# domanovi/FEC_Erasure_Code_Unit_Test_Relay

Hardware: AMD Instinct MI355X
Metric: GiB/s device-resident erasure encode+decode, 300B pkts, T=10; %HBM roofline (higher is better)
Workload: dtype u8; 1 GPU; encode 1000010 + decode 1000000 x 300B packets per GPU, one stream per GPU, (T,B,N)=(10,3,3); T=10, B=3, N=3, packets_per_gpu=1000000

## Files before the change

fec_erasure_code_unit_test_relay_amd/_lib.py:

```python
from __future__ import annotations

import ctypes
import os

_HERE = os.path.dirname(os.path.abspath(__file__))
LIB_PATH = os.environ.get("FEC_AMD_LIB") or os.path.join(_HERE, "libfec_amd.so")
HEADER_PATHS = [os.path.join(_HERE, "..", "include", "fec_amd.h")]

FEC_OK = 0
FEC_ERR_ARG = -1
FEC_ERR_HIP = -2
FEC_ERR_NOMEM = -3
FEC_ERR_WORKSPACE = -4
FEC_ERR_SEQUENCE = -5
FEC_ERR_HISTORY = -6

KERNEL_NAMES = ["fec_encode_kernel", "fec_scan_kernel", "fec_plan_kernel", "fec_copy_kernel",
                "fec_recover_kernel"]


class FecError(RuntimeError):
    def __init__(self, status: int, what: str = ""):
        msg = lib().fec_strerror(status).decode() if _lib is not None else str(status)
        if status == FEC_ERR_HIP and _lib is not None:
# ... 6 lines not shown

_lib = None


def lib() -> ctypes.CDLL:
    global _lib
    if _lib is not None:
        return _lib
    if not os.path.exists(LIB_PATH):
        raise RuntimeError(
            f"{LIB_PATH} is missing: the HIP extension must be built first "
            "(make -C fec_erasure_code_unit_test_relay_amd/csrc); there is no fallback")
    try:
        import torch
    except ImportError:
        pass
    L = ctypes.CDLL(LIB_PATH)
    vp, i32, i64 = ctypes.c_void_p, ctypes.c_int, ctypes.c_int64
    ip = ctypes.POINTER(ctypes.c_int)
    i64p = ctypes.POINTER(ctypes.c_int64)
    L.fec_strerror.restype = ctypes.c_char_p
    L.fec_strerror.argtypes = [i32]
    L.fec_last_error.restype = i32
    L.fec_last_error.argtypes = [ctypes.c_char_p, ctypes.c_size_t]
    L.fec_version.restype = i32
    L.fec_codec_create.argtypes = [i32, i32, i32, i32, ctypes.POINTER(vp)]
    L.fec_codec_destroy.argtypes = [vp]
    L.fec_codec_geometry.argtypes = [vp, ip, ip, ip, ip]
    L.fec_codec_generator.argtypes = [vp, vp]
    L.fec_codec_set_encode_path.argtypes = [vp, i32]
    L.fec_encode_tile_fetch.argtypes = [i32, i32, i32, i32, i32, ip, ip, ip, ip]
    L.fec_codec_set_copy_path.argtypes = [vp, i32]
    L.fec_codec_set_plan_path.argtypes = [vp, i32]
    L.fec_codec_info.argtypes = [vp, ctypes.c_char_p, ctypes.c_size_t]
    L.fec_codec_set_episode_dedup.argtypes = [vp, i32]
    L.fec_debug_stamps.argtypes = [vp, i32, vp]
    L.fec_encode_batch.argtypes = [vp, vp, vp, i64, i64, vp, vp, vp]
    L.fec_decode_workspace_bytes.restype = ctypes.c_size_t
    L.fec_decode_workspace_bytes.argtypes = [vp, i64]
    L.fec_decode_batch.argtypes = [vp, vp, vp, i64, vp, vp, vp, ctypes.c_size_t, vp]
    L.fec_decode_counters.argtypes = [vp, i64p, i64p, i64p]
    L.fec_streams_create.argtypes = [i32, i32, i32, i32, i32, ctypes.POINTER(vp)]
    L.fec_streams_destroy.argtypes = [vp]
    L.fec_streams_encode.argtypes = [vp, vp, i32, vp, vp, vp, vp, vp]
    L.fec_streams_decode.argtypes = [vp, vp, i32, vp, vp, vp, vp, vp]
    L.fec_streams_state.argtypes = [vp, i32, i64p, i64p]
    L.fec_streams_encode_burst.argtypes = [vp, vp, vp, i32, vp, vp, vp, vp, vp]
    L.fec_streams_decode_burst.argtypes = [vp, vp, vp, i32, vp, vp, vp, vp, vp]
    L.fec_streams_plan_burst_host.argtypes = [i32, i32, i32, i32, vp, vp, i32, vp]
    L.fec_streams_create_mixed.argtypes = [i32, vp, i32, vp, i32, ctypes.POINTER(vp)]
    L.fec_streams_codes.argtypes = [vp, ip, ip]
    L.fec_streams_stream_geometry.argtypes = [vp, i32, ip, ip, ip, ip, ip, ip]
    L.fec_streams_set_code.argtypes = [vp, i32, i32]
    L.fec_streams_mixed_fit.argtypes = [i32, vp, i32, vp, vp, vp, vp]
    L.fec_decode_stream_create.argtypes = [ctypes.POINTER(vp)]
    L.fec_decode_stream_destroy.argtypes = [vp]
    L.fec_decode_stream_state.argtypes = [vp, i64p, i64p]
    L.fec_decode_stream_push.argtypes = [vp, vp, vp, vp, vp, i64, i64, vp, vp, i64p, vp, ctypes.c_size_t, vp]
    L.fec_decode_plan_stats.argtypes = [vp, i64p, i64p]
    L.fec_decode_plan.argtypes = [vp, vp, i64, vp, ctypes.c_size_t, vp]
    L.fec_decode_apply.argtypes = [vp, vp, vp, i64, vp, vp, vp, ctypes.c_size_t, vp]
    L.fec_decode_copy.argtypes = [vp, vp, vp, i64, vp, vp, vp]
    L.fec_decode_recover.argtypes = [vp, vp, i64, vp, vp, vp, ctypes.c_size_t, vp]
    L.fec_timing_enable.argtypes = [vp, i32]
    L.fec_timing_collect.argtypes = [vp, ctypes.POINTER(ctypes.c_double), i64p]
    L.fec_encoder_create.argtypes = [i32, i32, i32, i32, ctypes.POINTER(vp)]
# ... 119 lines not shown
```

fec_erasure_code_unit_test_relay_amd/codec.py:

```python
from __future__ import annotations

import ctypes

import numpy as np

from ._lib import KERNEL_NAMES, check, lib


def _stream_handle(torch):
    return ctypes.c_void_p(torch.cuda.current_stream().cuda_stream)


def _ptr(t):
    return ctypes.c_void_p(t.data_ptr()) if t is not None else None


def _check_out(torch, out, out_len, rows: int, width: int, device):
    if out is None:
        out = torch.empty((rows, width), dtype=torch.uint8, device=device)
    else:
        assert out.dtype == torch.uint8 and out.is_cuda and out.is_contiguous(), "out: contiguous uint8 GPU tensor"
        assert out.dim() == 2 and out.shape[1] == width and out.shape[0] >= rows, \
            f"out must be at least [{rows}, {width}], got {tuple(out.shape)}"
    if out_len is None:
# ... 14 lines not shown
class Codec:

    def __init__(self, max_payload: int, T: int, B: int, N: int):
        h = ctypes.c_void_p()
        check(lib().fec_codec_create(max_payload, T, B, N, ctypes.byref(h)), "fec_codec_create")
        self._h = h
        v = [ctypes.c_int() for _ in range(4)]
        check(lib().fec_codec_geometry(h, *[ctypes.byref(x) for x in v]), "fec_codec_geometry")
        self.k, self.n, self.S, self.CW = (x.value for x in v)
        self.L, self.T, self.B, self.N = max_payload, T, B, N
        self._ws = None

    def __del__(self):
        if getattr(self, "_h", None) and lib is not None:
            try:
                lib().fec_codec_destroy(self._h)
            except Exception:
                pass
            self._h = None

    def generator(self) -> np.ndarray:
        G = np.zeros(self.k * self.n, dtype=np.uint8)
        check(lib().fec_codec_generator(self._h, G.ctypes.data_as(ctypes.c_void_p)), "generator")
        return G.reshape(self.k, self.n)

    def set_encode_path(self, path: str) -> None:
        code = {"auto": 0, "generic": 1, "tile": 5}[path]
        check(lib().fec_codec_set_encode_path(self._h, code), "fec_codec_set_encode_path")

    def set_copy_path(self, path: str) -> None:
        code = {"auto": 0, "generic": 1, "fast": 2}[path]
        check(lib().fec_codec_set_copy_path(self._h, code), "fec_codec_set_copy_path")

    def info(self) -> dict:
        import json
        buf = ctypes.create_string_buffer(512)
        check(lib().fec_codec_info(self._h, buf, 512), "fec_codec_info")
        return json.loads(buf.value.decode())

    def set_plan_path(self, path: str) -> None:
        code = {"auto": 0, "generic": 1, "fast": 2}[path]
        check(lib().fec_codec_set_plan_path(self._h, code), "fec_codec_set_plan_path")

    def set_episode_dedup(self, on: bool) -> None:
        check(lib().fec_codec_set_episode_dedup(self._h, int(bool(on))), "fec_codec_set_episode_dedup")

    def encode_blocks(self, data, out=None):
        import torch
        assert data.dtype == torch.uint8 and data.is_cuda and data.dim() == 2 and data.shape[1] == self.k
        data = data.contiguous()
        if out is None:
            out = torch.empty((data.shape[0], self.n), dtype=torch.uint8, device=data.device)
        check(lib().fec_block_encode_batch(self._h, _ptr(data), data.shape[0], _ptr(out), _stream_handle(torch)),
              "fec_block_encode_batch")
        return out

    def decode_blocks(self, cw, erasure):
        import torch
        assert cw.dtype == torch.uint8 and cw.is_cuda and cw.dim() == 2 and cw.shape[1] == self.n
        assert erasure.dtype == torch.uint8 and erasure.shape == cw.shape
        cw, erasure = cw.contiguous(), erasure.contiguous()
        out = torch.empty_like(cw)
        er_out = torch.empty_like(erasure)
        check(lib().fec_block_decode_batch(self._h, _ptr(cw), _ptr(erasure), cw.shape[0], _ptr(out), _ptr(er_out),
                                           _stream_handle(torch)), "fec_block_decode_batch")
        return out, er_out

    def encode(self, payload, lengths=None, history: int = 0, out=None, out_len=None):
        import torch
        assert payload.dtype == torch.uint8 and payload.is_cuda and payload.dim() == 2
# ... 353 lines not shown
```

fec_erasure_code_unit_test_relay_amd/csrc/fec_codec.hip:

```cpp
#include <hip/hip_runtime.h>
#include <hip/hip_ext.h>

#include <algorithm>
#include <atomic>
#include <chrono>
#include <functional>
#include <cstdio>
#include <cstdlib>
#include <cstring>
#include <memory>
#include <mutex>
#include <new>
#include <vector>

#include "fec_amd.h"
#include "fec_host.h"
#include "fec_kernels.h"
#include "fec_status.h"

using fec::Geometry;

namespace {

constexpr int kLdsBudget = 64 * 1024;
constexpr int kCopyLdsBudget = 32 * 1024;
constexpr int kMaxPayload = 1500;

inline int round16(int v) { return (v + 15) & ~15; }

#define HIP_TRY(expr)                                  \
    do {                                               \
        if ((expr) != hipSuccess) return FEC_ERR_HIP;  \
    } while (0)

struct EventPair {
    int kernel;
    hipEvent_t a, b;
};

}

struct fec_decode_stream {
    int64_t consumed = 0;
    int64_t last_cut = 0;
};

struct fec_codec {
    Geometry g;
    bool compact_fresh = false;
    std::vector<uint8_t> G;
    std::shared_ptr<const fec::DecodeRules> rules;
    uint32_t* d_ptab = nullptr;
    uint8_t* d_rules = nullptr;
    int64_t* d_wbase = nullptr;
    uint8_t* d_rules_log = nullptr;
    const void* plan_fast = nullptr;
    uint8_t* d_gf = nullptr;
    uint8_t* d_G = nullptr;
    uint8_t* d_rstate = nullptr;
    int enc_tp = 0;
    int encode_path = 0;
    int cus = 0;
    const void* tile_kernel = nullptr;
    fec::TileGeom tile{};
    int tile_per_cu = 0;
    const void* copy_fast = nullptr;
    int copyf_tp = 0;
    int copy_path = 0;
    int plan_path = 0;
    int dedup = 1;
    uint64_t* d_stamps = nullptr;
    int stamp_kernel = -1;
    int copy_tp = 0;
    bool timing = false;
    std::vector<EventPair> events;
    hipStream_t side = nullptr;
    hipEvent_t ev_fork = nullptr, ev_join = nullptr;

    ~fec_codec() {
        if (ev_fork) (void)hipEventDestroy(ev_fork);
        if (ev_join) (void)hipEventDestroy(ev_join);
        if (side) (void)hipStreamDestroy(side);
        for (auto& e : events) {
            (void)hipEventDestroy(e.a);
            (void)hipEventDestroy(e.b);
        }
        if (d_ptab) (void)hipFree(d_ptab);
        if (d_rules) (void)hipFree(d_rules);
        if (d_wbase) (void)hipFree(d_wbase);
        if (d_rules_log) (void)hipFree(d_rules_log);
        if (d_gf) (void)hipFree(d_gf);
        if (d_G) (void)hipFree(d_G);
        if (d_rstate) (void)hipFree(d_rstate);
    }

    int enc_lds(int tp) const {
        const int SP = (g.S + 3) & ~3;
        const int rows = tp + g.n - 1;
        const int Sk = g.S * g.k;
        return round16(g.k * rows * SP) + round16(tp * g.CW) + 2 * ((Sk + 7) & ~7) + 4 * rows;
    }
    int copy_lds(int tp) const { return round16(tp * g.CW) + 2 * ((g.L + 2 + 7) & ~7) + 4 * tp; }
// ... 383 lines not shown
    ca.CW = g.CW;
    ca.T = g.T;
    ca.TP = c->copy_tp;
    ca.cwt_bytes = round16(ca.TP * g.CW);
    const int64_t cblocks = (Pout + ca.TP - 1) / ca.TP;
    hipEvent_t stop;
    if (int st = c->begin(FEC_KERNEL_DEC_COPY, s, &stop)) return st;
    hipLaunchKernelGGL(fec::fec_copy_kernel, dim3(static_cast<unsigned>(cblocks)), dim3(256),
                       c->copy_lds(ca.TP), s, ca);
    HIP_TRY(hipGetLastError());
    return c->end(stop, s);
}

int launch_compact(fec_codec* c, int64_t P, void* d_ws, size_t ws_bytes, hipStream_t s) {
    const Geometry& g = c->g;
    if (P - g.T <= 0) return FEC_OK;
    if (int st = check_ws(c, P, d_ws, ws_bytes)) return st;
    const Ws w = ws_carve(g, P, d_ws);
    fec::CompactArgs ca;
    ca.counters = w.counters;
    ca.erased = w.erased;
    ca.src_d = w.src_d;
    ca.sym_ok = w.sym_ok;
    ca.k = g.k;
    ca.rec_list = w.rec_list;
    if (!c->compact_fresh)
        HIP_TRY(hipMemsetAsync(w.counters + 2, 0, 4, s));
    c->compact_fresh = false;
    hipLaunchKernelGGL(fec::fec_compact_kernel, dim3(256), dim3(256), 0, s, ca);
    HIP_TRY(hipGetLastError());
    return FEC_OK;
}

int launch_recover(fec_codec* c, const uint8_t* d_cw, int64_t P, uint8_t* d_out, int32_t* d_outlen,
                   void* d_ws, size_t ws_bytes, hipStream_t s, int64_t row_off = 0, bool compacted = false) {
    const Geometry& g = c->g;
    const int64_t Pout = P - g.T;
    if (Pout <= 0) return FEC_OK;
    if (int st = check_ws(c, P, d_ws, ws_bytes)) return st;
    if (!compacted)
        if (int st = launch_compact(c, P, d_ws, ws_bytes, s)) return st;
    const Ws w = ws_carve(g, P, d_ws);
    fec::RecArgs ra;
    ra.cw = d_cw;
    ra.P = P;
    ra.Pout = Pout;
    ra.counters = w.counters;
    ra.rec_list = w.rec_list;
    ra.coef = w.coef;
    ra.gf = c->d_gf;
    ra.out = d_out;
    ra.out_len = d_outlen;
    ra.L = g.L;
    ra.k = g.k;
    ra.n = g.n;
    ra.S = g.S;
    ra.CW = g.CW;
    hipEvent_t stop;
    if (int st = c->begin(FEC_KERNEL_DEC_RECOVER, s, &stop)) return st;
    ra.row_off = row_off;
    ra.stamps = (c->stamp_kernel == FEC_KERNEL_DEC_RECOVER) ? c->d_stamps : nullptr;
    const int span = (g.k + g.n - 1) * g.CW + 32;
    ra.stage_bytes = (span <= 12 * 1024 && g.n <= 17) ? ((span + 15) & ~15) : 0;
    const unsigned rgrid = static_cast<unsigned>(std::min<int64_t>((Pout + 3) / 4, 1024));
    const int maxn = g.n <= 17 ? 17 : 32;
    const int lds = fec::recover_lds_bytes(maxn, ra.stage_bytes);
    if (g.n > 17)
        hipLaunchKernelGGL((fec::fec_recover_kernel_t<32, false>), dim3(rgrid), dim3(256), lds, s, ra);
    else if (ra.stage_bytes)
        hipLaunchKernelGGL((fec::fec_recover_kernel_t<17, true>), dim3(rgrid), dim3(256), lds, s, ra);
    else
        hipLaunchKernelGGL((fec::fec_recover_kernel_t<17, false>), dim3(rgrid), dim3(256), lds, s, ra);
    HIP_TRY(hipGetLastError());
    return c->end(stop, s);
}

int launch_decode(fec_codec* c, const uint8_t* d_cw, const uint8_t* d_er, int64_t P, uint8_t* d_out,
                  int32_t* d_outlen, void* d_ws, size_t ws_bytes, hipStream_t s) {
    if (P - c->g.T <= 0) return FEC_OK;
    if (int st = check_ws(c, P, d_ws, ws_bytes)) return st;
    HIP_TRY(hipEventRecord(c->ev_fork, s));
    HIP_TRY(hipStreamWaitEvent(c->side, c->ev_fork, 0));
    if (int st = launch_plan(c, d_er, P, d_ws, ws_bytes, c->side)) return st;
    if (int st = launch_compact(c, P, d_ws, ws_bytes, c->side)) return st;
    HIP_TRY(hipEventRecord(c->ev_join, c->side));
    if (int st = launch_copy(c, d_cw, d_er, P, d_out, d_outlen, s)) return st;
    HIP_TRY(hipStreamWaitEvent(s, c->ev_join, 0));
    return launch_recover(c, d_cw, P, d_out, d_outlen, d_ws, ws_bytes, s, 0, true);
}

int launch_decode_stream(fec_codec* c, fec_decode_stream* st, const uint8_t* d_cw, const uint8_t* d_er,
                         const uint8_t* h_er, int64_t P, int64_t history, uint8_t* d_out, int32_t* d_outlen,
                         int64_t* n_out, void* d_ws, size_t ws_bytes, hipStream_t s) {
    const int T = c->g.T;
// ... 300 lines not shown
    if (!c || P < 0) return FEC_ERR_ARG;
    if (P > c->g.T && (!d_cw || !d_out || !d_outlen)) return FEC_ERR_ARG;
    return launch_recover(c, d_cw, P, d_out, d_outlen, d_ws, ws_bytes,
                          static_cast<hipStream_t>(stream));
}

int fec_decode_counters(const void* d_ws, int64_t* episodes, int64_t* recovered, int64_t* lost) {
    if (!d_ws) return FEC_ERR_ARG;
    int32_t h[8];
    HIP_TRY(hipDeviceSynchronize());
    HIP_TRY(hipMemcpy(h, d_ws, sizeof(h), hipMemcpyDeviceToHost));
    if (episodes) *episodes = h[6] + h[7];
    if (recovered) *recovered = h[2];
    if (lost) *lost = h[1] - h[2];
    return FEC_OK;
}

int fec_codec_info(const fec_codec* c, char* buf, size_t size) {
    if (!c || !buf || size == 0) return FEC_ERR_ARG;
    char enc[64];
    const int np = c->g.n - c->g.k;
    if (c->tile_kernel && (c->encode_path == 0 || c->encode_path == 5))
        std::snprintf(enc, sizeof(enc), "fec_encode_tile_kernel<%d, %d, %d, false>", c->g.k, np,
                      c->tile_kernel == fec::fec_encode_tile_kernel_for(c->g.k, np, 0) ? 0 : c->g.L);
    else
        std::snprintf(enc, sizeof(enc), "fec_encode_kernel");
    char cpy[64];
    if (c->copy_path != 1 && copy_pair_kernel(c))
        std::snprintf(cpy, sizeof(cpy), "fec_copy_pair_kernel<%d, %d>", c->g.k, np);
    else if (c->copy_fast && c->copy_path != 1)
        std::snprintf(cpy, sizeof(cpy), "fec_copy_fast_kernel<%d, %d>", c->g.k, np);
    else
        std::snprintf(cpy, sizeof(cpy), "fec_copy_kernel");
    std::snprintf(buf, size,
                  "{\"k\": %d, \"n\": %d, \"S\": %d, \"CW\": %d, \"encode_kernel\": \"%s\", "
                  "\"copy_kernel\": \"%s\", \"encode_tile_packets\": %d, \"encode_tile_workgroups_per_cu\": %d, "
                  "\"copy_tile\": %d, \"plan_specialised\": %d}",
                  c->g.k, c->g.n, c->g.S, c->g.CW, enc, cpy, c->tile.R, c->tile_per_cu, c->copyf_tp,
                  c->plan_fast ? 1 : 0);
    return FEC_OK;
}

int fec_decode_plan_stats(const void* d_ws, int64_t* replayed, int64_t* filled) {
    if (!d_ws) return FEC_ERR_ARG;
    int32_t h[8];
    HIP_TRY(hipDeviceSynchronize());
    HIP_TRY(hipMemcpy(h, d_ws, sizeof(h), hipMemcpyDeviceToHost));
    if (replayed) *replayed = h[6];
    if (filled) *filled = h[7];
    return FEC_OK;
}

int fec_debug_stamps(fec_codec* c, int kernel, void* d_stamps) {
    if (!c) return FEC_ERR_ARG;
    c->stamp_kernel = d_stamps ? kernel : -1;
    c->d_stamps = static_cast<uint64_t*>(d_stamps);
    return FEC_OK;
}

int fec_codec_set_episode_dedup(fec_codec* c, int on) {
    if (!c) return FEC_ERR_ARG;
    c->dedup = on ? 1 : 0;
    return FEC_OK;
}

int fec_codec_set_plan_path(fec_codec* c, int path) {
    if (!c || path < 0 || path > 2) return FEC_ERR_ARG;
    if (path == 2 && !c->plan_fast) return FEC_ERR_ARG;
    c->plan_path = path;
    return FEC_OK;
}

int fec_codec_set_copy_path(fec_codec* c, int path) {
    if (!c || path < 0 || path > 2) return FEC_ERR_ARG;
    if (path == 2 && !c->copy_fast) return FEC_ERR_ARG;
    c->copy_path = path;
    return FEC_OK;
}

int fec_codec_set_encode_path(fec_codec* c, int path) {
    if (!c || !(path == 0 || path == 1 || path == 5)) return FEC_ERR_ARG;
    if (path == 5 && !c->tile_kernel) return FEC_ERR_ARG;
    c->encode_path = path;
    return FEC_OK;
}

int fec_encode_tile_fetch(int max_payload, int T, int B, int N, int seg, int* R, int* issued, int* live_body,
                          int* live_front) {
    if (max_payload < 0 || T < 0 || B < 0 || N < 0 || N > T) return FEC_ERR_ARG;
    const int L = max_payload, k = T - N + 1, np = B, n = k + np;
    const fec::TileGeom tg = fec::tile_geometry(k, np, L, seg != 0);
    const bool have = (L & 3) == 0 && tg.ok &&
                      (seg ? fec::fec_encode_tile_seg_kernel_for(k, np, L) : fec::fec_encode_tile_kernel_for(k, np, L));
    int body = 0, front = 0;
    if (have) {
        const int CPR = (L + 15) >> 4;
        for (int c = 0; c < tg.ngl * 256; ++c) {
            body += fec::tile_piece_live(tg.R, CPR, n, c, false);
            front += np > 0 && fec::tile_piece_live(tg.R, CPR, n, c, true);
        }
    }
    if (R) *R = have ? tg.R : 0;
    if (issued) *issued = have ? tg.ngl * 256 : 0;
    if (live_body) *live_body = body;
    if (live_front) *live_front = front;
    return have ? 1 : 0;
}

int fec_timing_enable(fec_codec* c, int enable) {
    if (!c) return FEC_ERR_ARG;
// ... 615 lines not shown
```

fec_erasure_code_unit_test_relay_amd/csrc/fec_copy_fast.hip:

```cpp
#include "fec_device.h"
#include "fec_kernels.h"

namespace fec {

template <int K, int NP>
__device__ __forceinline__ void copy_tile_convert(const CopyFastArgs& a, int64_t x0, int ntile, int delta,
                                                  const uint8_t* raw, uint8_t* xo, int32_t* clen, const uint8_t* erw) {
    constexpr int n = K + NP;
    const int tid = threadIdx.x, NT = blockDim.x;
    const int L = a.L, CW = a.CW, NS4 = a.NS4, T = a.T;
    for (int t = tid; t < ntile; t += NT) {
        int ln = 0, copy = 0;
        if (!erw[t]) {
            const uint8_t* row = raw + delta + t * CW;
            const int hdr = row[0] * 256 + row[(1 / K) * n + 1 % K];
            bool slow = false;
            for (int d = 0; d <= T; ++d) slow = slow || erw[t + d];
            ln = slow ? min(hdr, L) : hdr;
            copy = min(ln, L);
        }
        clen[t] = copy;
        a.out_len[x0 + t] = ln;
    }
    __syncthreads();
// ... 99 lines not shown
            if (lo >= delta && lo + 16 <= total) *reinterpret_cast<uint4*>(raw + lo) = v[q];
        }
        if (tid == 0) {
            for (int b = delta; b < total && (b & 3); ++b) raw[b] = gA[b];
            for (int b = total & ~3; b < total && b >= ((delta + 3) & ~3); ++b) raw[b] = gA[b];
        }
        for (int o = tid * 4; o < 32; o += 256 * 4) {
            const int lo16 = delta & ~15, hi16 = total & ~15;
            const int oa = lo16 + o, ob = hi16 + (o - 16);
            if (o < 16 && oa >= delta && oa + 4 <= total && !(lo16 >= delta && lo16 + 16 <= total))
                *reinterpret_cast<uint32_t*>(raw + oa) = *reinterpret_cast<const uint32_t*>(gA + oa);
            if (o >= 16 && ob >= delta && ob + 4 <= total && hi16 != lo16)
                *reinterpret_cast<uint32_t*>(raw + ob) = *reinterpret_cast<const uint32_t*>(gA + ob);
        }
        for (int i = tid; i < ntile + T; i += 256) erw[i] = a.er[x0 + i];
    };
    const int64_t xa = static_cast<int64_t>(blockIdx.x) * 2 * a.TP, xb = xa + a.TP;
    const int na = static_cast<int>(min<int64_t>(a.TP, a.Pout - xa));
    const int nb = static_cast<int>(max<int64_t>(0, min<int64_t>(a.TP, a.Pout - xb)));
    const int da = static_cast<int>(reinterpret_cast<uintptr_t>(a.cw + xa * CW) & 15);
    const int db = static_cast<int>(reinterpret_cast<uintptr_t>(a.cw + xb * CW) & 15);
    load(xa, na, da);
    land(xa, na, da);
    __syncthreads();
    if (nb > 0) load(xb, nb, db);
    copy_tile_convert<K, NP>(a, xa, na, da, raw, xo, clen, erw);
    if (nb <= 0) return;
    __syncthreads();
    land(xb, nb, db);
    __syncthreads();
    copy_tile_convert<K, NP>(a, xb, nb, db, raw, xo, clen, erw);
}

#define FEC_COPY_FAST_LIST(X) \
    X(8, 3) X(9, 5) X(11, 0) X(10, 1) X(9, 2) X(7, 4) X(6, 5) X(5, 6) X(4, 7) X(3, 8) X(2, 9)  \
    X(1, 10) X(10, 3) X(9, 3) X(10, 4) X(8, 4) X(10, 5) X(7, 5) X(3, 9)

#define FEC_COPY_FAST_INST(K, NP) \
    template __global__ void fec_copy_fast_kernel<K, NP>(CopyFastArgs); \
    template __global__ void fec_copy_pair_kernel<K, NP>(CopyFastArgs);
FEC_COPY_FAST_LIST(FEC_COPY_FAST_INST)

const void* fec_copy_pair_kernel_for(int k, int np) {
#define FEC_COPY_PAIR_CASE(K, NP) \
    if (k == K && np == NP) return reinterpret_cast<const void*>(&fec_copy_pair_kernel<K, NP>);
    FEC_COPY_FAST_LIST(FEC_COPY_PAIR_CASE)
#undef FEC_COPY_PAIR_CASE
    return nullptr;
}

const void* fec_copy_fast_kernel_for(int k, int np) {
#define FEC_COPY_FAST_CASE(K, NP) \
    if (k == K && np == NP) return reinterpret_cast<const void*>(&fec_copy_fast_kernel<K, NP>);
    FEC_COPY_FAST_LIST(FEC_COPY_FAST_CASE)
#undef FEC_COPY_FAST_CASE
    return nullptr;
}

}
```

fec_erasure_code_unit_test_relay_amd/csrc/fec_kernels.h:

```cpp
#pragma once

#include <hip/hip_runtime.h>
#include <cstddef>
#include <stdint.h>

namespace fec {

struct EncArgs {
    const uint8_t* payload;
    const int32_t* len;
    int64_t history;
    int64_t P;
    uint8_t* cw;
    int32_t* cw_len;
    const uint32_t* ptab;
    int L, k, n, S, CW;
    int SP;
    int TP;
    int ROWS;
    int plane;
    int xin_bytes, xout_bytes;
};

struct TileGeom {
// ... 80 lines not shown
struct EncMultiArgs {
    const uint8_t* payload;
    const int32_t* len;
    const uint32_t* gtab;
    const int64_t* seg;
    uint8_t* cur_rows;
    uint8_t* old_rows;
    int32_t* cur_len;
    int32_t* old_len;
    int L;
    int ntuple;
    int tkey[kEncMultiMax];
    int tfirst[kEncMultiMax + 1];
    int toff[kEncMultiMax];
    int nt;
    int ncf;
    int cf_first;
};
bool fec_encode_tile_multi_supports(int k, int np, int L);
const void* fec_encode_tile_multi_kernel_ptr();

struct CopyFastArgs {
    const uint8_t* cw;
    const uint8_t* er;
    int64_t P, Pout;
    uint8_t* out;
    int32_t* out_len;
    int L, CW, NS4, T, TP;
    int raw_bytes;
    int out_bytes;
    uint64_t* stamps;
};

const void* fec_copy_fast_kernel_for(int k, int np);
constexpr int kPairQ = 6;
const void* fec_copy_pair_kernel_for(int k, int np);
const void* fec_plan_fast_kernel_for(int k, int np);

struct CopyArgs {
    const uint8_t* cw;
    const uint8_t* er;
    int64_t P, Pout;
    uint8_t* out;
    int32_t* out_len;
    int L, k, n, S, CW, T, TP;
    int cwt_bytes;
};

constexpr int kPlanMaxN = 31;

struct PlanArgs {
    const uint8_t* er;
    int64_t P, Pout;
    const uint8_t* rules;
    const uint8_t* G;
    int64_t wbase[kPlanMaxN + 1];
    const uint8_t* gf;
    int ES;
    int k, n, T;
    const int32_t* counters;
    const int32_t* work;
    const int32_t* dups;
    const uint64_t* keys;
    const int32_t* reps_tr;
    int32_t* src_d;
    const uint8_t* rstate;
// ... 26 lines not shown
    uint64_t* stamps;
};
__global__ void fec_episode_kernel(EpisodeArgs a);

struct CompactArgs {
    int32_t* counters;
    const int32_t* erased;
    const int32_t* src_d;
    const uint8_t* sym_ok;
    int k;
    int32_t* rec_list;
};
__global__ void fec_compact_kernel(CompactArgs a);

struct RecArgs {
    const uint8_t* cw;
    int64_t P, Pout;
    const int32_t* counters;
    const int32_t* rec_list;
    const uint8_t* coef;
    const uint8_t* gf;
    uint8_t* out;
    int32_t* out_len;
    int L, k, n, S, CW;
    int64_t row_off;
    int stage_bytes;
    uint64_t* stamps;
};
inline int recover_lds_bytes(int maxn, int stage_bytes) {
    return 1552 + 4 * (((2 * 16 * maxn + 15) & ~15) + stage_bytes);
}
template <int MAXN, bool STAGED>
__global__ void fec_recover_kernel_t(RecArgs a);


struct BlockArgs {
    const uint8_t* in;
    const uint8_t* er;
    uint8_t* out;
    uint8_t* er_out;
    int64_t nblk;
    int k, n;
    const uint8_t* G;
    const uint8_t* gf;
    const uint8_t* rules;
    int64_t wbase_n;
    int ES;
};
__global__ void fec_block_encode_kernel(BlockArgs a);

struct CodecView {
    int L, T, B, N, k, n, S, CW;
    const uint8_t* G;
    const uint8_t* gf;
    const uint8_t* rules;
    int64_t wbase_n;
    int ES;
    const uint32_t* ptab;
};
__global__ void fec_block_decode_kernel(BlockArgs a);

__global__ void fec_encode_kernel(EncArgs a);
__global__ void fec_plan_kernel(PlanArgs a);
__global__ void fec_copy_kernel(CopyArgs a);

__global__ void fec_fill_kernel(uint8_t* out, int64_t t0, int64_t count, int L, uint64_t seed);
// ... 54 lines not shown
```

include/fec_amd.h:

```cpp
#ifndef FEC_AMD_H
#define FEC_AMD_H

#include <stddef.h>
#include <stdint.h>

#ifdef __cplusplus
extern "C" {
#endif

#define FEC_OK 0
#define FEC_ERR_ARG (-1)
#define FEC_ERR_HIP (-2)
#define FEC_ERR_NOMEM (-3)
#define FEC_ERR_WORKSPACE (-4)
#define FEC_ERR_SEQUENCE (-5)
#define FEC_ERR_HISTORY (-6)

typedef struct fec_codec fec_codec;
typedef struct fec_encoder fec_encoder;
typedef struct fec_decoder fec_decoder;

#define FEC_AMD_ABI_VERSION 2

const char *fec_strerror(int status);
int fec_last_error(char *buf, size_t size);
int fec_version(void);

int fec_codec_create(int max_payload, int T, int B, int N, fec_codec **out);
int fec_codec_destroy(fec_codec *codec);
int fec_codec_geometry(const fec_codec *codec, int *k, int *n, int *S, int *CW);
int fec_codec_info(const fec_codec *codec, char *buf, size_t size);
int fec_codec_set_encode_path(fec_codec *codec, int path);
int fec_encode_tile_fetch(int max_payload, int T, int B, int N, int seg, int *R, int *issued, int *live_body,
                          int *live_front);
int fec_codec_set_copy_path(fec_codec *codec, int path);
int fec_codec_set_plan_path(fec_codec *codec, int path);
int fec_codec_set_episode_dedup(fec_codec *codec, int on);
int fec_codec_generator(const fec_codec *codec, uint8_t *G);

int fec_encode_batch(fec_codec *codec, const uint8_t *d_payload, const int32_t *d_payload_len,
                     int64_t history, int64_t P, uint8_t *d_codeword, int32_t *d_codeword_len,
                     void *hip_stream);

size_t fec_decode_workspace_bytes(const fec_codec *codec, int64_t P);
int fec_decode_batch(fec_codec *codec, const uint8_t *d_codeword, const uint8_t *d_erasure,
                     int64_t P, uint8_t *d_payload_out, int32_t *d_payload_len, void *d_workspace,
                     size_t workspace_bytes, void *hip_stream);
typedef struct fec_decode_stream fec_decode_stream;
int fec_decode_stream_create(fec_decode_stream **out);
int fec_decode_stream_destroy(fec_decode_stream *st);
int fec_decode_stream_push(fec_codec *codec, fec_decode_stream *st, const uint8_t *d_codeword,
                           const uint8_t *d_erasure, const uint8_t *h_erasure, int64_t P, int64_t history,
                           uint8_t *d_payload_out, int32_t *d_payload_len, int64_t *n_out,
                           void *d_workspace, size_t workspace_bytes, void *hip_stream);
int fec_decode_stream_state(const fec_decode_stream *st, int64_t *consumed, int64_t *last_cut);
int fec_decode_plan(fec_codec *codec, const uint8_t *d_erasure, int64_t P, void *d_workspace,
                    size_t workspace_bytes, void *hip_stream);
int fec_decode_apply(fec_codec *codec, const uint8_t *d_codeword, const uint8_t *d_erasure,
                     int64_t P, uint8_t *d_payload_out, int32_t *d_payload_len, void *d_workspace,
                     size_t workspace_bytes, void *hip_stream);
int fec_decode_copy(fec_codec *codec, const uint8_t *d_codeword, const uint8_t *d_erasure,
                    int64_t P, uint8_t *d_payload_out, int32_t *d_payload_len, void *hip_stream);
int fec_decode_recover(fec_codec *codec, const uint8_t *d_codeword, int64_t P,
                       uint8_t *d_payload_out, int32_t *d_payload_len, void *d_workspace,
                       size_t workspace_bytes, void *hip_stream);
int fec_decode_counters(const void *d_workspace, int64_t *episodes, int64_t *recovered,
                        int64_t *lost);
int fec_decode_plan_stats(const void *d_ws, int64_t *replayed, int64_t *filled);
// ... 204 lines not shown
```

Baseline: 979.7 GiB/s.

## Add specialised one-wave-per-row erasure recover kernel with LDS staging and GF tables

Adds a templated fast recover kernel, specialised per (k, n-k). Each 64-lane wave stages one recovered row's codeword span into LDS with 16-byte vector loads, prefetches the next row's indices, and builds per-coefficient nibble multiply tables in LDS. It then computes four output bytes per lane with packed GF(256) table multiplies and writes the output with aligned 32-bit stores. The aim is to cut the per-byte gather and GF multiply cost of the generic recover kernel. In exchange it adds template instantiations and only applies when the span fits the staging buffer. The generic path stays selectable.

```diff
diff --git a/fec_erasure_code_unit_test_relay_amd/_lib.py b/fec_erasure_code_unit_test_relay_amd/_lib.py
--- a/fec_erasure_code_unit_test_relay_amd/_lib.py
+++ b/fec_erasure_code_unit_test_relay_amd/_lib.py
@@ -62,6 +62,12 @@
     L.fec_encode_tile_fetch.argtypes = [i32, i32, i32, i32, i32, ip, ip, ip, ip]
     L.fec_codec_set_copy_path.argtypes = [vp, i32]
     L.fec_codec_set_plan_path.argtypes = [vp, i32]
+    L.fec_codec_set_recover_path.argtypes = [vp, i32]
+    L.fec_codec_set_recover_path.restype = i32
+    L.fec_recover_fast_items.argtypes = [i32, i32, i32, i32, i64, i64, vp, vp, vp]
+    L.fec_recover_fast_items.restype = i32
+    L.fec_recover_fast_mul.argtypes = [ctypes.c_uint32, ctypes.c_uint32]
+    L.fec_recover_fast_mul.restype = ctypes.c_uint32
     L.fec_codec_info.argtypes = [vp, ctypes.c_char_p, ctypes.c_size_t]
     L.fec_codec_set_episode_dedup.argtypes = [vp, i32]
     L.fec_debug_stamps.argtypes = [vp, i32, vp]
diff --git a/fec_erasure_code_unit_test_relay_amd/codec.py b/fec_erasure_code_unit_test_relay_amd/codec.py
--- a/fec_erasure_code_unit_test_relay_amd/codec.py
+++ b/fec_erasure_code_unit_test_relay_amd/codec.py
@@ -70,10 +70,14 @@
         code = {"auto": 0, "generic": 1, "fast": 2}[path]
         check(lib().fec_codec_set_copy_path(self._h, code), "fec_codec_set_copy_path")
 
+    def set_recover_path(self, path: str) -> None:
+        code = {"auto": 0, "generic": 1, "fast": 2}[path]
+        check(lib().fec_codec_set_recover_path(self._h, code), "fec_codec_set_recover_path")
+
     def info(self) -> dict:
         import json
-        buf = ctypes.create_string_buffer(512)
-        check(lib().fec_codec_info(self._h, buf, 512), "fec_codec_info")
+        buf = ctypes.create_string_buffer(1024)
+        check(lib().fec_codec_info(self._h, buf, 1024), "fec_codec_info")
         return json.loads(buf.value.decode())
 
     def set_plan_path(self, path: str) -> None:
diff --git a/fec_erasure_code_unit_test_relay_amd/csrc/fec_codec.hip b/fec_erasure_code_unit_test_relay_amd/csrc/fec_codec.hip
--- a/fec_erasure_code_unit_test_relay_amd/csrc/fec_codec.hip
+++ b/fec_erasure_code_unit_test_relay_amd/csrc/fec_codec.hip
@@ -16,6 +16,7 @@
 #include "fec_amd.h"
 #include "fec_host.h"
 #include "fec_kernels.h"
+#include "fec_recover_fast.h"
 #include "fec_status.h"
 
 using fec::Geometry;
@@ -68,6 +69,7 @@
     int copyf_tp = 0;
     int copy_path = 0;
     int plan_path = 0;
+    int recover_path = 0;
     int dedup = 1;
     uint64_t* d_stamps = nullptr;
     int stamp_kernel = -1;
@@ -517,6 +519,11 @@
     return FEC_OK;
 }
 
+const void* recover_fast_kernel(const Geometry& g) {
+    if (fec::rec_fast_span_max(g.k, g.n, g.CW) > fec::kRecFastStageMax) return nullptr;
+    return fec::fec_recover_fast_kernel_for(g.k, g.n - g.k);
+}
+
 int launch_recover(fec_codec* c, const uint8_t* d_cw, int64_t P, uint8_t* d_out, int32_t* d_outlen,
                    void* d_ws, size_t ws_bytes, hipStream_t s, int64_t row_off = 0, bool compacted = false) {
     const Geometry& g = c->g;
@@ -545,6 +552,16 @@
     if (int st = c->begin(FEC_KERNEL_DEC_RECOVER, s, &stop)) return st;
     ra.row_off = row_off;
     ra.stamps = (c->stamp_kernel == FEC_KERNEL_DEC_RECOVER) ? c->d_stamps : nullptr;
+    if (c->recover_path != 0 && c->recover_path != 1 && c->recover_path != 2) return FEC_ERR_ARG;
+    const void* fk = recover_fast_kernel(g);
+    if (c->recover_path == 2 && !fk) return FEC_ERR_ARG;
+    if (fk && c->recover_path != 1) {
+        ra.stage_bytes = round16(fec::rec_fast_span_max(g.k, g.n, g.CW));
+        void* args[] = {&ra};
+        HIP_TRY(hipLaunchKernel(fk, dim3(static_cast<unsigned>(fec::rec_fast_waves(Pout))), dim3(64), args,
+                                fec::recover_fast_lds_bytes(g.k, g.n, ra.stage_bytes, g.L), s));
+        return c->end(stop, s);
+    }
     const int span = (g.k + g.n - 1) * g.CW + 32;
     ra.stage_bytes = (span <= 12 * 1024 && g.n <= 17) ? ((span + 15) & ~15) : 0;
     const unsigned rgrid = static_cast<unsigned>(std::min<int64_t>((Pout + 3) / 4, 1024));
@@ -911,12 +928,20 @@
         std::snprintf(cpy, sizeof(cpy), "fec_copy_fast_kernel<%d, %d>", c->g.k, np);
     else
         std::snprintf(cpy, sizeof(cpy), "fec_copy_kernel");
+    char rec[64];
+    const bool rfast = c->recover_path != 1 && recover_fast_kernel(c->g);
+    if (rfast)
+        std::snprintf(rec, sizeof(rec), "fec_recover_fast_kernel<%d, %d>", c->g.k, np);
+    else
+        std::snprintf(rec, sizeof(rec), "fec_recover_kernel_t<%d, %s>", c->g.n <= 17 ? 17 : 32,
+                      c->g.n <= 17 && (c->g.k + c->g.n - 1) * c->g.CW + 32 <= 12 * 1024 ? "true" : "false");
     std::snprintf(buf, size,
                   "{\"k\": %d, \"n\": %d, \"S\": %d, \"CW\": %d, \"encode_kernel\": \"%s\", "
                   "\"copy_kernel\": \"%s\", \"encode_tile_packets\": %d, \"encode_tile_workgroups_per_cu\": %d, "
-                  "\"copy_tile\": %d, \"plan_specialised\": %d}",
+                  "\"copy_tile\": %d, \"plan_specialised\": %d, \"recover_kernel\": \"%s\", "
+                  "\"recover_waves\": %d, \"recover_wave_rows\": %d}",
                   c->g.k, c->g.n, c->g.S, c->g.CW, enc, cpy, c->tile.R, c->tile_per_cu, c->copyf_tp,
-                  c->plan_fast ? 1 : 0);
+                  c->plan_fast ? 1 : 0, rec, rfast ? fec::kRecFastMaxWaves : 4096, rfast ? fec::kRecFastWaveRows : 1);
     return FEC_OK;
 }
 
@@ -955,6 +980,51 @@
     if (path == 2 && !c->copy_fast) return FEC_ERR_ARG;
     c->copy_path = path;
     return FEC_OK;
+}
+
+int fec_codec_set_recover_path(fec_codec* c, int path) {
+    if (!c || path < 0 || path > 2) return FEC_ERR_ARG;
+    if (path == 2 && !recover_fast_kernel(c->g)) return FEC_ERR_ARG;
+    c->recover_path = path;
+    return FEC_OK;
+}
+
+int fec_recover_fast_items(int max_payload, int T, int B, int N, int64_t P, int64_t x, int64_t* span,
+                           int64_t* src_off, int32_t* out_idx) {
+    if (max_payload < 1 || T < 0 || B < 0 || N < 1 || N > T || B < N || P < 0) return FEC_ERR_ARG;
+    if (T - N + 1 > fec::kMaxK || T - N + 1 + B > fec::kMaxN - 1) return 0;
+    const Geometry g = Geometry::make(max_payload, T, B, N);
+    if (!recover_fast_kernel(g)) return 0;
+    const int items = g.k * ((g.S + 3) / 4);
+    if (!span) return items;
+    if (x < 0 || x >= P - T) return FEC_ERR_ARG;
+    const fec::RecFastSpan sp = fec::rec_fast_span(x, g.k, g.n, g.CW, P);
+    span[0] = sp.rlo;
+    span[1] = sp.rhi;
+    span[2] = sp.a0;
+    span[3] = std::min<int64_t>(sp.a0 + 16 * static_cast<int64_t>(sp.nb), P * g.CW);
+    span[4] = round16(fec::rec_fast_span_max(g.k, g.n, g.CW));
+    if (!src_off || !out_idx) return items;
+    for (int it = 0; it < items; ++it) {
+        const fec::RecFastItem m = fec::rec_fast_item(sp, x, it, g.k, g.n, g.S, g.CW, P);
+        for (int q = 0; q < g.n; ++q)
+            for (int e = 0; e < 4; ++e) {
+                const bool use = q >= m.qlo && q < m.qhi && e < m.ne;
+                src_off[(static_cast<int64_t>(it) * g.n + q) * 4 + e] =
+                    use ? sp.a0 + m.base + q * (g.CW + 1) + e * g.n : -1;
+            }
+        for (int e = 0; e < 4; ++e) {
+            const int h = (4 * m.g + e) * g.k + m.i;
+            out_idx[it * 4 + e] = (e < m.ne && h < g.L + 2) ? h : -1;
+        }
+    }
+    return items;
+}
+
+uint32_t fec_recover_fast_mul(uint32_t c, uint32_t x4) {
+    uint32_t tab[5];
+    fec::gf_mul4x_tables(c, tab);
+    return fec::gf_mul4x_portable(tab, x4);
 }
 
 int fec_codec_set_encode_path(fec_codec* c, int path) {
diff --git a/fec_erasure_code_unit_test_relay_amd/csrc/fec_copy_fast.hip b/fec_erasure_code_unit_test_relay_amd/csrc/fec_copy_fast.hip
--- a/fec_erasure_code_unit_test_relay_amd/csrc/fec_copy_fast.hip
+++ b/fec_erasure_code_unit_test_relay_amd/csrc/fec_copy_fast.hip
@@ -155,10 +155,6 @@
     copy_tile_convert<K, NP>(a, xb, nb, db, raw, xo, clen, erw);
 }
 
-#define FEC_COPY_FAST_LIST(X) \
-    X(8, 3) X(9, 5) X(11, 0) X(10, 1) X(9, 2) X(7, 4) X(6, 5) X(5, 6) X(4, 7) X(3, 8) X(2, 9)  \
-    X(1, 10) X(10, 3) X(9, 3) X(10, 4) X(8, 4) X(10, 5) X(7, 5) X(3, 9)
-
 #define FEC_COPY_FAST_INST(K, NP) \
     template __global__ void fec_copy_fast_kernel<K, NP>(CopyFastArgs); \
     template __global__ void fec_copy_pair_kernel<K, NP>(CopyFastArgs);
diff --git a/fec_erasure_code_unit_test_relay_amd/csrc/fec_kernels.h b/fec_erasure_code_unit_test_relay_amd/csrc/fec_kernels.h
--- a/fec_erasure_code_unit_test_relay_amd/csrc/fec_kernels.h
+++ b/fec_erasure_code_unit_test_relay_amd/csrc/fec_kernels.h
@@ -136,6 +136,10 @@
     uint64_t* stamps;
 };
 
+#define FEC_COPY_FAST_LIST(X) \
+    X(8, 3) X(9, 5) X(11, 0) X(10, 1) X(9, 2) X(7, 4) X(6, 5) X(5, 6) X(4, 7) X(3, 8) X(2, 9)  \
+    X(1, 10) X(10, 3) X(9, 3) X(10, 4) X(8, 4) X(10, 5) X(7, 5) X(3, 9)
+
 const void* fec_copy_fast_kernel_for(int k, int np);
 constexpr int kPairQ = 6;
 const void* fec_copy_pair_kernel_for(int k, int np);
@@ -228,6 +232,10 @@
 }
 template <int MAXN, bool STAGED>
 __global__ void fec_recover_kernel_t(RecArgs a);
+const void* fec_recover_fast_kernel_for(int k, int np);
+inline int recover_fast_lds_bytes(int k, int n, int stage_bytes, int L) {
+    return ((20 * k * n + 15) & ~15) + stage_bytes + ((L + 16 + 15) & ~15);
+}
 
 
 struct BlockArgs {
diff --git a/fec_erasure_code_unit_test_relay_amd/csrc/fec_recover_fast.h b/fec_erasure_code_unit_test_relay_amd/csrc/fec_recover_fast.h
--- /dev/null
+++ b/fec_erasure_code_unit_test_relay_amd/csrc/fec_recover_fast.h
@@ -0,0 +1,87 @@
+#pragma once
+
+#include <hip/hip_runtime.h>
+#include <stdint.h>
+
+namespace fec {
+
+constexpr int kRecFastStageChunks = 12;
+constexpr int kRecFastStageMax = kRecFastStageChunks * 64 * 16;
+constexpr int kRecFastWaveRows = 16;
+constexpr int kRecFastMaxWaves = 4096;
+
+__host__ __device__ inline int rec_fast_span_max(int k, int n, int CW) { return (k + n - 1) * CW + 32; }
+
+__host__ __device__ inline int rec_fast_waves(int64_t Pout) {
+    const int64_t w = (Pout + kRecFastWaveRows - 1) / kRecFastWaveRows;
+    return static_cast<int>(w < 1 ? 1 : (w > kRecFastMaxWaves ? kRecFastMaxWaves : w));
+}
+
+struct RecFastSpan {
+    int rlo, rhi;
+    int64_t s0, s1, a0;
+    int nb;
+};
+__host__ __device__ inline RecFastSpan rec_fast_span(int64_t x, int k, int n, int CW, int64_t P) {
+    RecFastSpan sp;
+    sp.rlo = static_cast<int>(x - k + 1 > 0 ? x - k + 1 : 0);
+    sp.rhi = static_cast<int>(x + n < P ? x + n : P);
+    sp.s0 = static_cast<int64_t>(sp.rlo) * CW;
+    sp.s1 = static_cast<int64_t>(sp.rhi) * CW;
+    sp.a0 = sp.s0 & ~int64_t(15);
+    sp.nb = static_cast<int>((sp.s1 - sp.a0 + 15) >> 4);
+    return sp;
+}
+
+struct RecFastItem {
+    int i, g, ne, qlo, qhi, base;
+};
+__host__ __device__ inline RecFastItem rec_fast_item(const RecFastSpan& sp, int64_t x, int it, int k, int n, int S,
+                                                     int CW, int64_t P) {
+    RecFastItem m;
+    m.g = it / k;
+    m.i = it - m.g * k;
+    m.ne = S - 4 * m.g < 4 ? S - 4 * m.g : 4;
+    m.qlo = static_cast<int>(m.i - x > 0 ? m.i - x : 0);
+    const int64_t qh = P - x + m.i;
+    m.qhi = static_cast<int>(qh < n ? (qh > 0 ? qh : 0) : n);
+    m.base = static_cast<int>((x - m.i - sp.rlo) * CW + (sp.s0 - sp.a0)) + 4 * m.g * n;
+    return m;
+}
+
+__host__ __device__ inline uint32_t gf_double4(uint32_t v) {
+    const uint32_t hi = (v >> 7) & 0x01010101u;
+    return ((v & 0x7f7f7f7fu) << 1) ^ (hi * 0x1du);
+}
+__host__ __device__ inline uint32_t splat_byte1(uint32_t v) {
+    const uint32_t b = (v >> 8) & 0xffu;
+    const uint32_t h = b | (b << 8);
+    return h | (h << 16);
+}
+__host__ __device__ inline void gf_mul4x_tables(uint32_t c, uint32_t tab[5]) {
+    c &= 0xffu;
+    const uint32_t c2 = gf_double4(c);
+    const uint32_t t0 = (c << 8) | (c2 << 16) | ((c ^ c2) << 24);
+    const uint32_t t4 = gf_double4(gf_double4(t0));
+    const uint32_t t8 = gf_double4(t4);
+    const uint32_t t32 = gf_double4(gf_double4(t8));
+    const uint32_t t64 = gf_double4(t32);
+    tab[0] = t0;
+    tab[1] = t0 ^ splat_byte1(t4);
+    tab[2] = t8;
+    tab[3] = t8 ^ splat_byte1(t32);
+    tab[4] = t64;
+}
+__host__ __device__ inline uint32_t gf_mul4x_portable(const uint32_t tab[5], uint32_t x) {
+    uint32_t r = 0;
+    for (int e = 0; e < 4; ++e) {
+        const uint32_t b = (x >> (8 * e)) & 0xffu;
+        const uint32_t g0 = b & 7u, g1 = (b >> 3) & 7u, g2 = b >> 6;
+        const uint32_t p = ((tab[g0 >> 2] >> (8 * (g0 & 3))) ^ (tab[2 + (g1 >> 2)] >> (8 * (g1 & 3))) ^
+                            (tab[4] >> (8 * g2))) & 0xffu;
+        r |= p << (8 * e);
+    }
+    return r;
+}
+
+}
diff --git a/fec_erasure_code_unit_test_relay_amd/csrc/fec_recover_fast.hip b/fec_erasure_code_unit_test_relay_amd/csrc/fec_recover_fast.hip
--- /dev/null
+++ b/fec_erasure_code_unit_test_relay_amd/csrc/fec_recover_fast.hip
@@ -0,0 +1,130 @@
+#include "fec_device.h"
+#include "fec_kernels.h"
+#include "fec_recover_fast.h"
+
+namespace fec {
+
+template <int K, int NP>
+__global__ __launch_bounds__(64) void fec_recover_fast_kernel(RecArgs a) {
+    constexpr int n = K + NP;
+    constexpr int KN = K * n;
+    constexpr int kCf = (KN + 63) / 64;
+    extern __shared__ __attribute__((aligned(16))) uint8_t fsm[];
+    uint4* t4 = reinterpret_cast<uint4*>(fsm);
+    uint32_t* t1 = reinterpret_cast<uint32_t*>(fsm + 16 * KN);
+    uint8_t* rows = fsm + ((20 * KN + 15) & ~15);
+    uint8_t* obuf = rows + a.stage_bytes;
+    const int lane = threadIdx.x;
+    const int L = a.L, S = a.S, CW = a.CW;
+    const int NS4 = (S + 3) >> 2;
+    const int waves = gridDim.x;
+    const int64_t cw_total = a.P * CW;
+    phase_stamp(a.stamps, blockIdx.x, 0);
+    int r = blockIdx.x;
+    int nrec = a.counters[2];
+    int x = 0, xr = 0;
+    if (r < a.Pout) {
+        x = a.rec_list[2 * r];
+        xr = a.rec_list[2 * r + 1];
+    }
+    phase_stamp(a.stamps, blockIdx.x, 1);
+    while (r < nrec) {
+        const int rn = r + waves;
+        int xn = 0, xrn = 0;
+        if (rn < nrec) {
+            xn = a.rec_list[2 * rn];
+            xrn = a.rec_list[2 * rn + 1];
+        }
+        if (x >= a.row_off) {
+            uint8_t* orow = a.out + static_cast<int64_t>(x - a.row_off) * L;
+            const RecFastSpan sp = rec_fast_span(x, K, n, CW, a.P);
+            uint4 piece[kRecFastStageChunks];
+#pragma unroll
+            for (int j = 0; j < kRecFastStageChunks; ++j) {
+                const int c = lane + 64 * j;
+                const int64_t o = sp.a0 + 16 * c;
+                piece[j] = make_uint4(0u, 0u, 0u, 0u);
+                if (c < sp.nb && o + 16 <= cw_total) piece[j] = *reinterpret_cast<const uint4*>(a.cw + o);
+            }
+            const int ctail = static_cast<int>((cw_total - sp.a0) >> 4);
+            const bool tail = ctail < sp.nb;
+            uint32_t tbyte = 0;
+            if (tail && sp.a0 + 16 * ctail + lane < cw_total && lane < 16) tbyte = a.cw[sp.a0 + 16 * ctail + lane];
+            uint32_t cf[kCf];
+            const uint8_t* cfp = a.coef + static_cast<int64_t>(xr) * KN;
+#pragma unroll
+            for (int j = 0; j < kCf; ++j) cf[j] = lane + 64 * j < KN ? cfp[lane + 64 * j] : 0u;
+#pragma unroll
+            for (int j = 0; j < kRecFastStageChunks; ++j)
+                if (lane + 64 * j < sp.nb) *reinterpret_cast<uint4*>(rows + 16 * (lane + 64 * j)) = piece[j];
+            if (tail && lane < 16) rows[16 * ctail + lane] = static_cast<uint8_t>(tbyte);
+#pragma unroll
+            for (int j = 0; j < kCf; ++j) {
+                if (lane + 64 * j < KN) {
+                    uint32_t tab[5];
+                    gf_mul4x_tables(cf[j], tab);
+                    t4[lane + 64 * j] = make_uint4(tab[0], tab[1], tab[2], tab[3]);
+                    t1[lane + 64 * j] = tab[4];
+                }
+            }
+            __builtin_amdgcn_fence(__ATOMIC_RELEASE, "wavefront");
+            __builtin_amdgcn_wave_barrier();
+            __builtin_amdgcn_fence(__ATOMIC_ACQUIRE, "wavefront");
+            for (int it = lane; it < K * NS4; it += 64) {
+                const RecFastItem m = rec_fast_item(sp, x, it, K, n, S, CW, a.P);
+                const int o1 = m.ne > 1 ? n : 0, o2 = m.ne > 2 ? 2 * n : 0, o3 = m.ne > 3 ? 3 * n : 0;
+                uint32_t acc = 0;
+#pragma unroll
+                for (int q = 0; q < n; ++q) {
+                    const bool use = q >= m.qlo && q < m.qhi;
+                    const uint8_t* p = rows + (use ? m.base + q * (CW + 1) : 0);
+                    const uint32_t v = static_cast<uint32_t>(p[0]) | (static_cast<uint32_t>(p[o1]) << 8) |
+                                       (static_cast<uint32_t>(p[o2]) << 16) | (static_cast<uint32_t>(p[o3]) << 24);
+                    const uint4 ta = t4[m.i * n + q];
+                    const uint32_t tab[5] = {ta.x, ta.y, ta.z, ta.w, t1[m.i * n + q]};
+                    acc ^= gf_mul4x(tab, use ? v : 0u);
+                }
+#pragma unroll
+                for (int e = 0; e < 4; ++e) {
+                    const int h = (4 * m.g + e) * K + m.i;
+                    if (e < m.ne && h < L + 2) obuf[2 + h] = static_cast<uint8_t>(acc >> (8 * e));
+                }
+            }
+            __builtin_amdgcn_fence(__ATOMIC_RELEASE, "wavefront");
+            __builtin_amdgcn_wave_barrier();
+            __builtin_amdgcn_fence(__ATOMIC_ACQUIRE, "wavefront");
+            const int ln = min(static_cast<int>(obuf[2]) * 256 + static_cast<int>(obuf[3]), L);
+            const uint8_t* pl = obuf + 4;
+            const int head = min(L, static_cast<int>((4 - (reinterpret_cast<uintptr_t>(orow) & 3)) & 3));
+            const int nd = (L - head) >> 2;
+            const int tail0 = head + 4 * nd;
+            for (int w = lane; w < nd; w += 64) {
+                const int b = head + 4 * w;
+                const uint32_t lo = *reinterpret_cast<const uint32_t*>(pl + (b & ~3));
+                const uint32_t hi = *reinterpret_cast<const uint32_t*>(pl + (b & ~3) + 4);
+                *reinterpret_cast<uint32_t*>(orow + b) = __builtin_amdgcn_alignbyte(hi, lo, head) & keep_bytes(ln - b);
+            }
+            if (lane < head) orow[lane] = lane < ln ? pl[lane] : 0;
+            if (lane < L - tail0) orow[tail0 + lane] = tail0 + lane < ln ? pl[tail0 + lane] : 0;
+            if (lane == 0) a.out_len[x - a.row_off] = ln;
+            __builtin_amdgcn_wave_barrier();
+        }
+        r = rn;
+        x = xn;
+        xr = xrn;
+    }
+    phase_stamp(a.stamps, blockIdx.x, 2);
+}
+
+#define FEC_RECOVER_FAST_INST(K, NP) template __global__ void fec_recover_fast_kernel<K, NP>(RecArgs);
+FEC_COPY_FAST_LIST(FEC_RECOVER_FAST_INST)
+
+const void* fec_recover_fast_kernel_for(int k, int np) {
+#define FEC_RECOVER_FAST_CASE(K, NP) \
+    if (k == K && np == NP) return reinterpret_cast<const void*>(&fec_recover_fast_kernel<K, NP>);
+    FEC_COPY_FAST_LIST(FEC_RECOVER_FAST_CASE)
+#undef FEC_RECOVER_FAST_CASE
+    return nullptr;
+}
+
+}
diff --git a/include/fec_amd.h b/include/fec_amd.h
--- a/include/fec_amd.h
+++ b/include/fec_amd.h
@@ -34,6 +34,10 @@
 int fec_encode_tile_fetch(int max_payload, int T, int B, int N, int seg, int *R, int *issued, int *live_body,
                           int *live_front);
 int fec_codec_set_copy_path(fec_codec *codec, int path);
+int fec_codec_set_recover_path(fec_codec *codec, int path);
+int fec_recover_fast_items(int max_payload, int T, int B, int N, int64_t P, int64_t x, int64_t *span,
+                           int64_t *src_off, int32_t *out_idx);
+uint32_t fec_recover_fast_mul(uint32_t c, uint32_t x4);
 int fec_codec_set_plan_path(fec_codec *codec, int path);
 int fec_codec_set_episode_dedup(fec_codec *codec, int on);
 int fec_codec_generator(const fec_codec *codec, uint8_t *G);
```

Result: faster. 994.0 GiB/s, median of 6 (+1.5%).
